# zenghjian/SceneSplat

Measured on AMD Instinct MI355X. Metric: Gaussians/s encoder fwd+bwd, 102k-pt chunks, higher is better.
Workload: dtype bf16

## Files before the change

### include/scenesplat_hip.h

```cpp
#ifndef SCENESPLAT_HIP_H
#define SCENESPLAT_HIP_H
#include <stddef.h>
#include <stdint.h>

#ifdef __cplusplus
extern "C" {
#endif

struct ihipStream_t;
typedef struct ihipStream_t* ss_stream_t;

#define SS_MAX_ORDERS 8
enum { SS_ORDER_Z = 0, SS_ORDER_Z_TRANS = 1, SS_ORDER_HILBERT = 2, SS_ORDER_HILBERT_TRANS = 3 };
enum { SS_DTYPE_F32 = 0, SS_DTYPE_BF16 = 1 };
enum { SS_ATTN_SIMT = 0, SS_ATTN_MFMA = 1 };
enum { SS_OK = 0, SS_ERR_ARG = 1, SS_ERR_LAUNCH = 2, SS_ERR_WORKSPACE = 3 };

int ss_version(void);

int ss_serialize_encode(const int32_t* grid_coord, const int32_t* batch, int64_t n, int depth, const int* orders,
                        int num_orders, int64_t* codes, ss_stream_t stream);
int ss_offsets_to_batch(const int32_t* offsets, int num_batches, int64_t n, int32_t* batch, ss_stream_t stream);
int ss_count_duplicates(const int64_t* sorted_keys, int64_t n, int32_t* count, ss_stream_t stream);
int ss_grid_coord_max(const int32_t* grid_coord, int64_t n, int32_t* out_max, ss_stream_t stream);
// ... 60 lines not shown
size_t ss_window_attn_hm_bwd_workspace_bytes(int64_t n, int64_t n_pad, int channels, int num_heads);
int ss_window_attn_hm_bwd(const void* hm, const void* out, const void* dout, const float* neg_lse2, const int32_t* gidx,
                          const int32_t* sidx, const int32_t* win_start, int num_windows, int max_window, int64_t n,
                          int64_t n_pad, int channels, int num_heads, float scale, void* dqkv, void* workspace,
                          size_t workspace_bytes, ss_stream_t stream);

int ss_window_attn_rpe_fwd(const void* qkv, const int32_t* gidx, const int32_t* sidx, const int32_t* win_start,
                           int num_windows, int max_window, int64_t n, int64_t n_pad, int channels, int num_heads,
                           float scale, int dtype, int impl, const int32_t* grid_coord, const float* table, int pos_bnd,
                           void* out, float* lse, ss_stream_t stream);
size_t ss_window_attn_rpe_bwd_workspace_bytes(int64_t n, int64_t n_pad, int channels, int num_heads, int dtype,
                                              int num_windows, int max_window, int pos_bnd);
int ss_window_attn_rpe_bwd(const void* qkv, const void* out, const void* dout, const float* lse, const int32_t* gidx,
                           const int32_t* sidx, const int32_t* win_start, int num_windows, int max_window, int64_t n,
                           int64_t n_pad, int channels, int num_heads, float scale, int dtype, int impl,
                           const int32_t* grid_coord, const float* table, int pos_bnd, void* dqkv, float* dtable,
                           void* workspace, size_t workspace_bytes, ss_stream_t stream);

int ss_subm_rulebook(const int32_t* grid_coord, const int32_t* batch, int64_t n, int depth,
                     const int64_t* zkeys_sorted, const int32_t* zorder, int swap_xy, int kernel_size, int32_t* nbr,
                     ss_stream_t stream);
int ss_subm_tap_mask_keys(const int32_t* nbr, const int32_t* order, int64_t n, int taps, int coarse_bits, int64_t* keys,
                          ss_stream_t stream);
int64_t ss_subm_rulebook_table_size(int64_t n);
int ss_subm_rulebook_hashed(const int32_t* grid_coord, const int32_t* batch, int64_t n, int depth, int kernel_size, int32_t* nbr,
                            void* workspace, size_t workspace_bytes, ss_stream_t stream);

int ss_subm_conv_fwd(const void* in, const void* weight, const float* bias, const int32_t* nbr, const int32_t* rowperm,
                     void* out, int64_t n, int cin, int cout, int taps, int out_dtype, ss_stream_t stream);
int ss_subm_weight_mirror(const void* w, void* wt, int cout, int taps, int cin, ss_stream_t stream);
int ss_stream_create_cu_mask(int nwords, const uint32_t* mask, void** stream_out);
int ss_subm_im2col(const void* src, const int32_t* nbr, void* dst, int64_t n, int taps, int64_t row_bytes, ss_stream_t stream);
int ss_gemm8_ok(int64_t m, int k, int n, int taps);
int ss_subm_conv_fwd_pipe(const void* in, const void* weight, const float* bias, const int32_t* nbr, const int32_t* rowperm,
                          void* out, int64_t n, int cin, int cout, int taps, int out_dtype, ss_stream_t stream);
int ss_subm_conv_fwd_pipe_walk(const void* in, const void* weight, const float* bias, const int32_t* nbr_walk, const int32_t* rowperm,
                               void* out, int64_t n, int cin, int cout, int taps, int out_dtype, ss_stream_t stream);
int ss_subm_conv_fwd_uses_pipe(int64_t n, int cin, int cout, int taps);
int ss_subm_conv_fwd_walk(const void* in, const void* weight, const float* bias, const int32_t* nbr, const int32_t* nbr_walk,
                          const int32_t* rowperm, void* out, int64_t n, int cin, int cout, int taps, int out_dtype, ss_stream_t stream);
int ss_linear_fwd(const void* x, const void* weight, const float* bias, void* out, int64_t m, int k, int n, int out_dtype,
                  ss_stream_t stream);
int ss_wgrad_xcd_order(void);
int ss_wgrad_set_xcd_order(int on);
int ss_wgrad8_ok(int64_t n, int cin, int cout, int taps);
int ss_subm_conv_wgrad_pipe(const void* in, const void* dout, const int32_t* nbr, const int32_t* rowperm,
                            const int32_t* blk_count, const int32_t* blk_list, float* dweight, int64_t n, int cin, int cout,
                            int taps, ss_stream_t stream);
int ss_linear_wgrad(const void* x, const void* dy, float* dweight, float* dbias, int64_t m, int k_in, int n_out,
                    ss_stream_t stream);
int ss_linear_wgrad_group_plan(int64_t m, int k_in, int n_out, int64_t* desc_words);
int ss_linear_wgrad_tiles(int k_in, int n_out);
int ss_linear_wgrad_group_plan2(int64_t m, int k_in, int n_out, int launch_tiles, int64_t* desc_words);
int ss_linear_wgrad_group(const int64_t* desc, const int32_t* wg_start, int nprob, int total_workgroups, ss_stream_t stream);
int ss_subm_conv_splits(int64_t n, int cout, int taps);
int ss_subm_conv_fwd_splitk(const void* in, const void* weight, const float* bias, const int32_t* nbr, const int32_t* rowperm,
                            float* acc32, int64_t n, int cin, int cout, int taps, int splits, ss_stream_t stream);
int ss_subm_block_lists(const int32_t* nbr, const int32_t* rowperm, int64_t n, int taps, int32_t* blk_count,
                        int32_t* blk_list, ss_stream_t stream);
int ss_subm_conv_wgrad(const void* in, const void* dout, const int32_t* nbr, const int32_t* rowperm,
                       const int32_t* blk_count, const int32_t* blk_list, float* dweight, int64_t n, int cin, int cout,
                       int taps, ss_stream_t stream);

int ss_subm_f32_ok(int cin_padded, int cout);
int ss_subm_f32_fwd(const float* in, const float* wq, const float* bias, const int32_t* nbr_walk, const int32_t* rowperm,
                    float* out, int64_t n, int cin_padded, int cout, int taps, ss_stream_t stream);
int ss_subm_f32_dgrad_dup(const float* dout_folded, const float* wq, const int32_t* nbr_walk, const int32_t* rowperm, float* din,
                          int64_t n, int cin_padded, int cout, int taps, ss_stream_t stream);
int ss_subm_f32_wgrad(const float* in, const float* dout, const int32_t* nbr_walk, const int32_t* rowperm,
                      const int32_t* blk_count, const int32_t* blk_list, float* dweight, int64_t n, int cin_padded,
                      int cin, int cout, int taps, ss_stream_t stream);

int ss_subm_conv_wgrad_pipe_walk(const void* in, const void* dout, const int32_t* nbr_walk, const int32_t* rowperm,
                                 const int32_t* blk_count, const int32_t* blk_list, float* dweight, int64_t n, int cin, int cout,
                                 int taps, ss_stream_t stream);
int ss_subm_conv_wgrad_uses_pipe(int64_t n, int cin, int cout, int taps);
// ... 211 lines not shown
```

### scenesplat_amd/csrc/gemm8.hip

```cpp
#include "common.h"
#include <stdlib.h>

typedef __attribute__((ext_vector_type(8))) __bf16 g8_bf8_t;
#define G8_MFMA(a, b, c) __builtin_amdgcn_mfma_f32_16x16x32_bf16((a), (b), (c), 0, 0, 0)
#define G8_TAPS_MAX 27
#define G8_ZERO_ELEMS 4096

#ifndef G8_STAGGER
#define G8_STAGGER 1
#endif
#define G8_BUF 65536
#define G8_HALF 16384
#define G8_OFF_B 32768
#define G8_OFF_NBR 131072
#define G8_OFF_ROWID (G8_OFF_NBR + G8_TAPS_MAX * 256 * 4)
#define G8_OFF_MASK (G8_OFF_ROWID + 1024)
#define G8_LDS_BYTES (G8_OFF_MASK + 16)

__device__ uint4 g8_zero[G8_ZERO_ELEMS / 8];

__device__ __forceinline__ void g8_glds16(const void* gsrc, char* lds_wave_base) {
  __builtin_amdgcn_global_load_lds((const __attribute__((address_space(1))) void*)gsrc,
                                   (__attribute__((address_space(3))) void*)lds_wave_base, 16, 0, 0);
}
__device__ __forceinline__ g8_bf8_t g8_lds(const char* p) {
  return __builtin_bit_cast(g8_bf8_t, *reinterpret_cast<const uint4*>(p));
}

template <bool GATHER, typename OutT, bool HM = false>
__global__ void __launch_bounds__(512)
k_gemm8(const unsigned short* __restrict__ A, const unsigned short* __restrict__ W, const float* __restrict__ bias,
        const int32_t* __restrict__ nbr, const int32_t* __restrict__ rowperm, OutT* __restrict__ out, int M, int K,
        int N, int taps, int ntn, int hm_c = 0, int hm_d = 0, float hm_scale = 1.f, int walk = 0) {
  __shared__ __attribute__((aligned(16))) char smem[G8_LDS_BYTES];
  int32_t* nbr_s = reinterpret_cast<int32_t*>(smem + G8_OFF_NBR);
  int32_t* rowid_s = reinterpret_cast<int32_t*>(smem + G8_OFF_ROWID);
  unsigned* mask_s = reinterpret_cast<unsigned*>(smem + G8_OFF_MASK);
  const int tid = threadIdx.x, wave = tid >> 6, lane = tid & 63, lq = lane & 15, g = lane >> 4;
  const int wr = wave >> 2, wc = wave & 3;
  int L;
  {
    const int nwg = gridDim.x, orig = blockIdx.x, xcd = orig & 7, q = nwg >> 3, r = nwg & 7;
    L = (xcd < r ? xcd * (q + 1) : r * (q + 1) + (xcd - r) * q) + (orig >> 3);
  }
  const int m0 = (L / ntn) * 256, n0 = (L % ntn) * 256;

  unsigned rem = 0u;
  int tap = 0;
  if (GATHER) {
    if (tid < 256) {
      int k = m0 + tid;
      rowid_s[tid] = k < M ? (rowperm ? rowperm[k] : k) : -1;
    }
    if (tid == 0) *mask_s = 0u;
    __syncthreads();
    constexpr int NIT = (G8_TAPS_MAX * 256 + 511) / 512;
    int vals[NIT];
    const int last = taps * 256 - 1;
#pragma unroll
    for (int it = 0; it < NIT; ++it) {
      const int e = min(it * 512 + tid, last), tt = e >> 8, r = e & 255;
      if (walk) {
        const int k = m0 + r;
        const int v = nbr[(int64_t)tt * M + min(k, M - 1)];
        vals[it] = k < M ? v : -1;
      } else {
        const int row = rowid_s[r];
        const int v = nbr[(int64_t)tt * M + max(row, 0)];
        vals[it] = row >= 0 ? v : -1;
      }
    }
#pragma unroll
    for (int it = 0; it < NIT; ++it) {
      const int e = it * 512 + tid;
      if (e <= last) {
        nbr_s[e] = vals[it];
        if (__ballot(vals[it] >= 0) != 0ULL && lane == 0) atomicOr(mask_s, 1u << (e >> 8));
      }
    }
    __syncthreads();
    rem = __builtin_amdgcn_readfirstlane(*mask_s);
  }
  const int ksteps = K >> 6;
  int T;
  if (GATHER) {
    T = __builtin_popcount(rem) * ksteps;
    if (rem) { tap = __builtin_ctz(rem); rem &= rem - 1u; }
  } else {
    T = ksteps;
  }

  f32x4_t acc[2][4][2][2];
#pragma unroll
  for (int a = 0; a < 2; ++a)
#pragma unroll
    for (int mi = 0; mi < 4; ++mi)
#pragma unroll
      for (int b = 0; b < 2; ++b)
#pragma unroll
        for (int ni = 0; ni < 2; ++ni) acc[a][mi][b][ni] = f32x4_t{0.f, 0.f, 0.f, 0.f};

  const int lc8 = (((tid & 7) ^ ((tid >> 4) & 7)) << 3);
  const int srow = tid >> 3;
  const unsigned short* pA[4];
  const unsigned short* pB[2][2];
  auto load_rows = [&](int tp) {
#pragma unroll
    for (int q = 0; q < 4; ++q) {
      int R = 128 * (q >> 1) + 64 * (q & 1) + srow;
      if (GATHER) {
        int src = nbr_s[tp * 256 + R];
        pA[q] = (src >= 0 ? A + (int64_t)src * K : reinterpret_cast<const unsigned short*>(g8_zero)) + lc8;
      } else {
        int row = min(m0 + R, M - 1);
        if (HM) row = rowperm[row];
        pA[q] = A + (int64_t)row * K + lc8;
      }
    }
  };
#pragma unroll
  for (int h = 0; h < 2; ++h)
#pragma unroll
    for (int j = 0; j < 2; ++j) {
      int col = min(n0 + 128 * j + 64 * (tid >> 8) + 32 * h + (srow & 31), N - 1);
      pB[h][j] = W + (int64_t)col * taps * K + lc8;
    }
  int kc = 0;
  int64_t boff = (int64_t)tap * K;
  load_rows(tap);
  int staged = 0;
  auto advance = [&]() {
    if (staged + 1 >= T) return;
    ++staged;
    kc += 64;
    if (GATHER) {
      if (kc == K) {
        kc = 0;
        tap = __builtin_ctz(rem); rem &= rem - 1u;
        boff = (int64_t)tap * K;
        load_rows(tap);
      }
    } else if (kc == K) {
      kc = 0;
    }
  };
  char* const dst0 = smem + wave * 1024;
  auto stageA = [&](int buf, int h) {
    char* d = dst0 + buf * G8_BUF + h * G8_HALF;
    g8_glds16(pA[h] + kc, d);
    g8_glds16(pA[2 + h] + kc, d + 8192);
  };
  auto stageB = [&](int buf, int h) {
    char* d = dst0 + buf * G8_BUF + G8_OFF_B + h * G8_HALF;
    g8_glds16(pB[h][0] + boff + kc, d);
    g8_glds16(pB[h][1] + boff + kc, d + 8192);
  };

  const int sw = (lq >> 1) & 7;
  const int oA = (wr * 64 + lq) * 128 + ((g ^ sw) << 4);
  const int oB = G8_OFF_B + (wc * 32 + lq) * 128 + ((g ^ sw) << 4);
  g8_bf8_t af[4][2], b0f[2][2], b1f[2][2];
  auto readA = [&](int buf, int h) {
    const char* base = smem + buf * G8_BUF + h * G8_HALF;
#pragma unroll
    for (int mi = 0; mi < 4; ++mi) {
      af[mi][0] = g8_lds(base + oA + mi * 2048);
      af[mi][1] = g8_lds(base + (oA ^ 64) + mi * 2048);
    }
  };
  auto readB = [&](int buf, int h, g8_bf8_t (&bf)[2][2]) {
    const char* base = smem + buf * G8_BUF + h * G8_HALF;
#pragma unroll
    for (int ni = 0; ni < 2; ++ni) {
      bf[ni][0] = g8_lds(base + oB + ni * 2048);
      bf[ni][1] = g8_lds(base + (oB ^ 64) + ni * 2048);
    }
  };
#define G8_MM(HA, HB, BF)                                                                         \
  _Pragma("unroll") for (int ks = 0; ks < 2; ++ks)                                                \
  _Pragma("unroll") for (int mi = 0; mi < 4; ++mi)                                                \
  _Pragma("unroll") for (int ni = 0; ni < 2; ++ni)                                                \
      acc[HA][mi][HB][ni] = G8_MFMA(BF[ni][ks], af[mi][ks], acc[HA][mi][HB][ni]);
#define G8_BAR() do { __builtin_amdgcn_sched_barrier(0); __builtin_amdgcn_s_barrier(); __builtin_amdgcn_sched_barrier(0); } while (0)
#define G8_COMPUTE_BEGIN() do { G8_BAR(); asm volatile("s_waitcnt lgkmcnt(0)" ::: "memory"); __builtin_amdgcn_sched_barrier(0); __builtin_amdgcn_s_setprio(1); } while (0)
#define G8_COMPUTE_END() do { __builtin_amdgcn_s_setprio(0); G8_BAR(); } while (0)

  if (T > 0) {
    stageB(0, 0); stageA(0, 0); stageB(0, 1); stageA(0, 1);
    advance();
    stageB(1, 0); stageA(1, 0); stageB(1, 1);
    asm volatile("s_waitcnt vmcnt(6)" ::: "memory");
    G8_BAR();
#if G8_STAGGER
    if (wr == 1) G8_BAR();
#endif
    for (int t = 0; t < T; ++t) {
      const int buf = t & 1;
      readB(buf, 0, b0f);
      __builtin_amdgcn_sched_barrier(0);
      readA(buf, 0);
      stageA(buf ^ 1, 1);
#if G8_STAGGER
      __builtin_amdgcn_sched_barrier(0);
      asm volatile("s_waitcnt lgkmcnt(8)" ::: "memory");
#endif
      G8_COMPUTE_BEGIN();
      G8_MM(0, 0, b0f)
      G8_COMPUTE_END();
      advance();
      readB(buf, 1, b1f);
      stageB(buf, 0);
      G8_COMPUTE_BEGIN();
      G8_MM(0, 1, b1f)
      G8_COMPUTE_END();
      readA(buf, 1);
      stageA(buf, 0);
      G8_COMPUTE_BEGIN();
      G8_MM(1, 1, b1f)
      G8_COMPUTE_END();
      stageB(buf, 1);
      asm volatile("s_waitcnt vmcnt(6)" ::: "memory");
      G8_COMPUTE_BEGIN();
      G8_MM(1, 0, b0f)
      G8_COMPUTE_END();
    }
#if G8_STAGGER
    if (wr == 0) G8_BAR();
#endif
    asm volatile("s_waitcnt vmcnt(0)" ::: "memory");
  }

  int64_t hm_base[2][2];
  float hm_mul[2][2];
  if (HM) {
#pragma unroll
    for (int hb = 0; hb < 2; ++hb)
#pragma unroll
      for (int ni = 0; ni < 2; ++ni) {
        const int col = min(n0 + 64 * wc + 32 * hb + 16 * ni + 4 * g, N - 4);
        const int sec = col / hm_c, cc = col - sec * hm_c, hd = cc / hm_d, dd = cc - hd * hm_d;
        hm_base[hb][ni] = ((int64_t)sec * (hm_c / hm_d) + hd) * M * hm_d + dd;
        hm_mul[hb][ni] = sec == 0 ? hm_scale : 1.f;
      }
  }
#pragma unroll
  for (int ha = 0; ha < 2; ++ha)
#pragma unroll
    for (int mi = 0; mi < 4; ++mi) {
      const int R = 128 * wr + 64 * ha + 16 * mi + lq;
      int64_t row;
      if (GATHER) { row = rowid_s[R]; } else { row = m0 + R < M ? m0 + R : -1; }
      if (row < 0) continue;
#pragma unroll
      for (int hb = 0; hb < 2; ++hb)
#pragma unroll
        for (int ni = 0; ni < 2; ++ni) {
          const int col = n0 + 64 * wc + 32 * hb + 16 * ni + 4 * g;
          if (col >= N) continue;
          f32x4_t v = acc[ha][mi][hb][ni];
          if (bias) { float4 bv = *reinterpret_cast<const float4*>(bias + col); v[0] += bv.x; v[1] += bv.y; v[2] += bv.z; v[3] += bv.w; }
          OutT* op = out + row * N + col;
          if (HM) {
            const float m_ = hm_mul[hb][ni];
            v[0] *= m_; v[1] *= m_; v[2] *= m_; v[3] *= m_;
            op = out + hm_base[hb][ni] + row * hm_d;
          }
          if (sizeof(OutT) == 2) {
            uint2 u; u.x = pack_bf16x2(v[0], v[1]); u.y = pack_bf16x2(v[2], v[3]);
            *reinterpret_cast<uint2*>(op) = u;
          } else {
            *reinterpret_cast<float4*>(op) = make_float4(v[0], v[1], v[2], v[3]);
          }
        }
    }
}

extern "C" int ss_gemm8_ok(int64_t m, int k, int n, int taps) {
  return m > 0 && m < (1LL << 31) && k >= 64 && (k & 63) == 0 && k <= G8_ZERO_ELEMS && n >= 4 && (n & 3) == 0 &&
         taps >= 1 && taps <= G8_TAPS_MAX;
}

template <bool GATHER>
static int g8_launch(const void* a, const void* w, const float* bias, const int32_t* nbr, const int32_t* rowperm, void* out,
                     int64_t m, int k, int n, int taps, int out_dtype, hipStream_t stream, int walk = 0) {
  if (!ss_gemm8_ok(m, k, n, taps)) return SS_ERR_ARG;
  const int ntm = ss_div_up(m, 256), ntn = ss_div_up(n, 256);
  dim3 grid(ntm * ntn), block(512);
  const unsigned short* A = (const unsigned short*)a; const unsigned short* Wp = (const unsigned short*)w;
  if (out_dtype == SS_BF16)
    SS_LAUNCH((k_gemm8<GATHER, unsigned short>), grid, block, 0, stream, A, Wp, bias, nbr, rowperm, (unsigned short*)out, (int)m, k, n, taps, ntn, 0, 0, 1.f, walk);
  else if (out_dtype == SS_F32)
    SS_LAUNCH((k_gemm8<GATHER, float>), grid, block, 0, stream, A, Wp, bias, nbr, rowperm, (float*)out, (int)m, k, n, taps, ntn, 0, 0, 1.f, walk);
  else
    return SS_ERR_ARG;
  return SS_OK;
}

extern "C" int ss_subm_conv_fwd_pipe(const void* in, const void* weight, const float* bias, const int32_t* nbr,
                                     const int32_t* rowperm, void* out, int64_t n, int cin, int cout, int taps,
                                     int out_dtype, hipStream_t stream) {
  if (n == 0) return SS_OK;
  return g8_launch<true>(in, weight, bias, nbr, rowperm, out, n, cin, cout, taps, out_dtype, stream);
}

extern "C" int ss_subm_conv_fwd_pipe_walk(const void* in, const void* weight, const float* bias, const int32_t* nbr_walk,
                                          const int32_t* rowperm, void* out, int64_t n, int cin, int cout, int taps,
                                          int out_dtype, hipStream_t stream) {
  if (n == 0) return SS_OK;
  return g8_launch<true>(in, weight, bias, nbr_walk, rowperm, out, n, cin, cout, taps, out_dtype, stream, 1);
}

extern "C" int ss_linear_fwd(const void* x, const void* weight, const float* bias, void* out, int64_t m, int k, int n,
                             int out_dtype, hipStream_t stream) {
  if (m == 0) return SS_OK;
  return g8_launch<false>(x, weight, bias, nullptr, nullptr, out, m, k, n, 1, out_dtype, stream);
}

extern "C" int ss_linear_fwd_headmajor(const void* x, const int32_t* row_index, const void* weight, const float* bias,
                                       void* out_hm, int64_t m, int k, int n_out, int channels, int head_dim,
                                       float sec0_scale, hipStream_t stream) {
  if (m == 0) return SS_OK;
  if (!ss_gemm8_ok(m, k, n_out, 1) || channels <= 0 || head_dim <= 0 || (head_dim & 3) || channels % head_dim || n_out % channels ||
      !row_index)
    return SS_ERR_ARG;
  const int ntm = ss_div_up(m, 256), ntn = ss_div_up(n_out, 256);
  dim3 grid(ntm * ntn), block(512);
  SS_LAUNCH((k_gemm8<false, unsigned short, true>), grid, block, 0, stream, (const unsigned short*)x, (const unsigned short*)weight,
            bias, (const int32_t*)nullptr, row_index, (unsigned short*)out_hm, (int)m, k, n_out, 1, ntn, channels, head_dim,
            sec0_scale);
  return SS_OK;
}
```

### scenesplat_amd/native.py

```python
import ctypes

import numpy as np
import torch

from . import _lib, grouped
from ._lib import check

_C = _lib.CONSTANTS
F32, BF16 = _C["SS_DTYPE_F32"], _C["SS_DTYPE_BF16"]
ATTN_SIMT, ATTN_MFMA = _C["SS_ATTN_SIMT"], _C["SS_ATTN_MFMA"]
HAVE_MFMA_ATTN = True
ORDER_IDS = {name: _C["SS_ORDER_" + name.upper().replace("-", "_")] for name in ("z", "z-trans", "hilbert", "hilbert-trans")}


def _p(t):
    return ctypes.c_void_p(t.data_ptr()) if t is not None else ctypes.c_void_p(0)


def _stream():
    return ctypes.c_void_p(torch.cuda.current_stream().cuda_stream)


def _req(t, dtype=None, name="tensor", shape=None):
    if not isinstance(t, torch.Tensor) or not t.is_cuda:
# ... 168 lines not shown
        check(lib().ss_subm_conv_fwd_splitk(_p(x), _p(w), _p(bias), _p(nbr), _p(rowperm), _p(acc), n, cin, cout, taps, splits,
                                            _stream()), "ss_subm_conv_fwd_splitk")
        return acc if out_dtype == torch.float32 else acc.to(out_dtype)
    out = torch.empty((n, cout), dtype=out_dtype, device=x.device)
    if nbr_walk is not None:
        _req(nbr_walk, torch.int32, "nbr_walk", (taps, n))
        check(lib().ss_subm_conv_fwd_walk(_p(x), _p(w), _p(bias), _p(nbr), _p(nbr_walk), _p(rowperm), _p(out), n, cin, cout, taps,
                                          dtype_code(out), _stream()), "ss_subm_conv_fwd_walk")
        return out
    check(lib().ss_subm_conv_fwd(_p(x), _p(w), _p(bias), _p(nbr), _p(rowperm), _p(out), n, cin, cout, taps,
                                 dtype_code(out), _stream()), "ss_subm_conv_fwd")
    return out


def subm_weight_mirror(w):
    cout, taps, cin = w.shape
    _req(w, torch.bfloat16, "w")
    wt = torch.empty((cin, taps, cout), dtype=torch.bfloat16, device=w.device)
    check(lib().ss_subm_weight_mirror(_p(w), _p(wt), cout, taps, cin, _stream()), "ss_subm_weight_mirror")
    return wt


def subm_im2col(x, nbr):
    n, c = x.shape
    taps = nbr.shape[0]
    _req(x, torch.bfloat16, "x"); _req(nbr, torch.int32, "nbr", (taps, n))
    if c % 8:
        raise RuntimeError("subm_im2col: channels must be a multiple of 8")
    out = torch.empty((n, taps * c), dtype=torch.bfloat16, device=x.device)
    check(lib().ss_subm_im2col(_p(x), _p(nbr), _p(out), n, taps, c * 2, _stream()), "ss_subm_im2col")
    return out


def subm_conv_fwd_pipe(x, w, bias, nbr, rowperm, out_dtype=torch.bfloat16):
    n, cin = x.shape
    cout, taps = w.shape[0], w.shape[1]
    out = torch.empty((n, cout), dtype=out_dtype, device=x.device)
    check(lib().ss_subm_conv_fwd_pipe(_p(x), _p(w), _p(bias), _p(nbr), _p(rowperm), _p(out), n, cin, cout, taps,
                                      dtype_code(out), _stream()), "ss_subm_conv_fwd_pipe")
    return out


def linear_fwd(x, w, bias=None, out_dtype=torch.bfloat16):
    m, k = x.shape
    n = w.shape[0]
    out = torch.empty((m, n), dtype=out_dtype, device=x.device)
    check(lib().ss_linear_fwd(_p(x), _p(w), _p(bias), _p(out), m, k, n, dtype_code(out), _stream()), "ss_linear_fwd")
    return out


def subm_block_lists(nbr, rowperm):
    taps, n = nbr.shape
    _req(nbr, torch.int32, "nbr")
    if rowperm is not None:
        _req(rowperm, torch.int32, "rowperm", (n,))
    nb = (n + 63) // 64
    cnt = torch.empty(taps, dtype=torch.int32, device=nbr.device)
    lst = torch.empty((taps, nb), dtype=torch.int32, device=nbr.device)
    check(lib().ss_subm_block_lists(_p(nbr), _p(rowperm), n, taps, _p(cnt), _p(lst), _stream()), "ss_subm_block_lists")
    return cnt, lst


_ARENA = {"buf": None, "off": 0}


def zero_arena_begin(numel, device):
    _ARENA["buf"] = torch.zeros(int(numel), dtype=torch.float32, device=device) if numel > 0 else None
    _ARENA["off"] = 0


def zeros_f32(numel, device):
    buf, off = _ARENA["buf"], _ARENA["off"]
    if buf is not None and buf.device == device and off + numel <= buf.numel():
        _ARENA["off"] = off + ((numel + 3) & ~3)
        return buf[off:off + numel]
    return torch.zeros(int(numel), dtype=torch.float32, device=device)


def subm_conv_wgrad(x, dout, nbr, rowperm, blocks, out=None, nbr_walk=None):
    n, cin = x.shape
    cout = dout.shape[1]
# ... 1354 lines not shown
```

Measured before the change: 2.909 million.

## Add two-phase software-pipelined main loop to gemm8 kernel as default

Adds a PH template parameter to the 256x256 MFMA GEMM kernel and a new two-phase K-loop schedule. Each iteration splits into two compute halves with interleaved LDS reads and global->LDS staging, using fewer barriers than the existing four-phase schedule. The two-phase path becomes the default and the four-phase path stays selectable through an env var or a setter. The different wait counts and stage ordering risk changing latency hiding or exposing more memory stalls.

Result: no change. 2.931 million, median of 6 (+0.7%).

```diff
diff --git a/include/scenesplat_hip.h b/include/scenesplat_hip.h
--- a/include/scenesplat_hip.h
+++ b/include/scenesplat_hip.h
@@ -126,6 +126,7 @@
 int ss_linear_fwd(const void* x, const void* weight, const float* bias, void* out, int64_t m, int k, int n, int out_dtype,
                   ss_stream_t stream);
 int ss_wgrad_xcd_order(void);
+int ss_gemm8_set_phases(int phases);
 int ss_wgrad_set_xcd_order(int on);
 int ss_wgrad8_ok(int64_t n, int cin, int cout, int taps);
 int ss_subm_conv_wgrad_pipe(const void* in, const void* dout, const int32_t* nbr, const int32_t* rowperm,
diff --git a/scenesplat_amd/csrc/gemm8.hip b/scenesplat_amd/csrc/gemm8.hip
--- a/scenesplat_amd/csrc/gemm8.hip
+++ b/scenesplat_amd/csrc/gemm8.hip
@@ -8,6 +8,9 @@
 
 #ifndef G8_STAGGER
 #define G8_STAGGER 1
+#endif
+#ifndef G8_PHASES_DEFAULT
+#define G8_PHASES_DEFAULT 2
 #endif
 #define G8_BUF 65536
 #define G8_HALF 16384
@@ -27,7 +30,7 @@
   return __builtin_bit_cast(g8_bf8_t, *reinterpret_cast<const uint4*>(p));
 }
 
-template <bool GATHER, typename OutT, bool HM = false>
+template <bool GATHER, typename OutT, bool HM = false, int PH = 2>
 __global__ void __launch_bounds__(512)
 k_gemm8(const unsigned short* __restrict__ A, const unsigned short* __restrict__ W, const float* __restrict__ bias,
         const int32_t* __restrict__ nbr, const int32_t* __restrict__ rowperm, OutT* __restrict__ out, int M, int K,
@@ -185,7 +188,7 @@
 #define G8_COMPUTE_BEGIN() do { G8_BAR(); asm volatile("s_waitcnt lgkmcnt(0)" ::: "memory"); __builtin_amdgcn_sched_barrier(0); __builtin_amdgcn_s_setprio(1); } while (0)
 #define G8_COMPUTE_END() do { __builtin_amdgcn_s_setprio(0); G8_BAR(); } while (0)
 
-  if (T > 0) {
+  if (T > 0 && PH == 4) {
     stageB(0, 0); stageA(0, 0); stageB(0, 1); stageA(0, 1);
     advance();
     stageB(1, 0); stageA(1, 0); stageB(1, 1);
@@ -229,6 +232,49 @@
 #endif
     asm volatile("s_waitcnt vmcnt(0)" ::: "memory");
   }
+  if (T > 0 && PH == 2) {
+    stageB(0, 0); stageA(0, 0); stageB(0, 1); stageA(0, 1);
+    advance();
+    stageA(1, 0); stageB(1, 0); stageB(1, 1);
+    asm volatile("s_waitcnt vmcnt(6)" ::: "memory");
+    G8_BAR();
+#if G8_STAGGER
+    if (wr == 1) G8_BAR();
+    if (wr == 1) __builtin_amdgcn_s_setprio(1);
+#endif
+    for (int t = 0; t < T; ++t) {
+      const int buf = t & 1;
+      readB(buf, 0, b0f);
+      readA(buf, 0);
+      readB(buf, 1, b1f);
+      __builtin_amdgcn_sched_barrier(0);
+      stageA(buf ^ 1, 1);
+      __builtin_amdgcn_sched_barrier(0);
+      asm volatile("s_waitcnt vmcnt(8) lgkmcnt(0)" ::: "memory");
+      G8_BAR();
+      G8_MM(0, 0, b0f)
+      G8_MM(0, 1, b1f)
+      G8_BAR();
+      advance();
+      readA(buf, 1);
+      __builtin_amdgcn_sched_barrier(0);
+      stageA(buf, 0);
+      __builtin_amdgcn_sched_barrier(0);
+      stageB(buf, 0);
+      stageB(buf, 1);
+      __builtin_amdgcn_sched_barrier(0);
+      asm volatile("s_waitcnt vmcnt(8) lgkmcnt(0)" ::: "memory");
+      G8_BAR();
+      G8_MM(1, 1, b1f)
+      G8_MM(1, 0, b0f)
+      G8_BAR();
+    }
+#if G8_STAGGER
+    if (wr == 0) G8_BAR();
+    __builtin_amdgcn_s_setprio(0);
+#endif
+    asm volatile("s_waitcnt vmcnt(0)" ::: "memory");
+  }
 
   int64_t hm_base[2][2];
   float hm_mul[2][2];
@@ -280,6 +326,22 @@
          taps >= 1 && taps <= G8_TAPS_MAX;
 }
 
+static int g8_phases_flag = -1;
+static int g8_phases() {
+  if (g8_phases_flag < 0) { const char* e = getenv("SS_GEMM8_PHASES"); g8_phases_flag = (e && atoi(e) == 4) ? 4 : G8_PHASES_DEFAULT; }
+  return g8_phases_flag;
+}
+extern "C" int ss_gemm8_set_phases(int phases) {
+  if (phases != 0 && phases != 2 && phases != 4) return SS_ERR_ARG;
+  g8_phases_flag = phases ? phases : -1;
+  return SS_OK;
+}
+#define G8_LAUNCH_PH(GATHER_, OutT_, HM_, ...)                                                              \
+  do {                                                                                                      \
+    if (g8_phases() == 4) SS_LAUNCH((k_gemm8<GATHER_, OutT_, HM_, 4>), grid, block, 0, stream, __VA_ARGS__); \
+    else SS_LAUNCH((k_gemm8<GATHER_, OutT_, HM_, 2>), grid, block, 0, stream, __VA_ARGS__);                 \
+  } while (0)
+
 template <bool GATHER>
 static int g8_launch(const void* a, const void* w, const float* bias, const int32_t* nbr, const int32_t* rowperm, void* out,
                      int64_t m, int k, int n, int taps, int out_dtype, hipStream_t stream, int walk = 0) {
@@ -288,9 +350,9 @@
   dim3 grid(ntm * ntn), block(512);
   const unsigned short* A = (const unsigned short*)a; const unsigned short* Wp = (const unsigned short*)w;
   if (out_dtype == SS_BF16)
-    SS_LAUNCH((k_gemm8<GATHER, unsigned short>), grid, block, 0, stream, A, Wp, bias, nbr, rowperm, (unsigned short*)out, (int)m, k, n, taps, ntn, 0, 0, 1.f, walk);
+    G8_LAUNCH_PH(GATHER, unsigned short, false, A, Wp, bias, nbr, rowperm, (unsigned short*)out, (int)m, k, n, taps, ntn, 0, 0, 1.f, walk);
   else if (out_dtype == SS_F32)
-    SS_LAUNCH((k_gemm8<GATHER, float>), grid, block, 0, stream, A, Wp, bias, nbr, rowperm, (float*)out, (int)m, k, n, taps, ntn, 0, 0, 1.f, walk);
+    G8_LAUNCH_PH(GATHER, float, false, A, Wp, bias, nbr, rowperm, (float*)out, (int)m, k, n, taps, ntn, 0, 0, 1.f, walk);
   else
     return SS_ERR_ARG;
   return SS_OK;
@@ -325,8 +387,8 @@
     return SS_ERR_ARG;
   const int ntm = ss_div_up(m, 256), ntn = ss_div_up(n_out, 256);
   dim3 grid(ntm * ntn), block(512);
-  SS_LAUNCH((k_gemm8<false, unsigned short, true>), grid, block, 0, stream, (const unsigned short*)x, (const unsigned short*)weight,
-            bias, (const int32_t*)nullptr, row_index, (unsigned short*)out_hm, (int)m, k, n_out, 1, ntn, channels, head_dim,
-            sec0_scale);
+  G8_LAUNCH_PH(false, unsigned short, true, (const unsigned short*)x, (const unsigned short*)weight,
+               bias, (const int32_t*)nullptr, row_index, (unsigned short*)out_hm, (int)m, k, n_out, 1, ntn, channels, head_dim,
+               sec0_scale, 0);
   return SS_OK;
 }
diff --git a/scenesplat_amd/native.py b/scenesplat_amd/native.py
--- a/scenesplat_amd/native.py
+++ b/scenesplat_amd/native.py
@@ -239,6 +239,10 @@
     out = torch.empty((m, n), dtype=out_dtype, device=x.device)
     check(lib().ss_linear_fwd(_p(x), _p(w), _p(bias), _p(out), m, k, n, dtype_code(out), _stream()), "ss_linear_fwd")
     return out
+
+
+def gemm8_set_phases(phases):
+    check(lib().ss_gemm8_set_phases(int(phases)), "ss_gemm8_set_phases")
 
 
 def subm_block_lists(nbr, rowperm):
```

## Add persistent linear GEMM kernel with cross-tile prefetch and split conv path

Applied to the files above, without the earlier changes.

Splits the gemm8 kernel into a gather-conv variant and a dense linear variant. The linear and head-major kernels now run persistently: the grid is capped at the CU count and each workgroup loops over tiles in XCD-aware order. The next tile's loads are staged during the current tile's tail, and row indices and bias are prefetched into LDS via async loads. This is meant to remove launch and tail bubbles and pipeline drains between tiles. The cost is more complex control flow, inline asm LDS reads, and less parallelism when tiles are few.

New measurement: 2.880 million before, 2.894 million after (median of 6 runs). About the same (+0.5%).

```diff
diff --git a/include/scenesplat_hip.h b/include/scenesplat_hip.h
--- a/include/scenesplat_hip.h
+++ b/include/scenesplat_hip.h
@@ -116,6 +116,10 @@
 int ss_stream_create_cu_mask(int nwords, const uint32_t* mask, void** stream_out);
 int ss_subm_im2col(const void* src, const int32_t* nbr, void* dst, int64_t n, int taps, int64_t row_bytes, ss_stream_t stream);
 int ss_gemm8_ok(int64_t m, int k, int n, int taps);
+int ss_gemm8_persistent(void);
+int ss_gemm8_set_persistent(int on);
+int ss_gemm8_max_wgs(void);
+int ss_gemm8_set_max_wgs(int cap);
 int ss_subm_conv_fwd_pipe(const void* in, const void* weight, const float* bias, const int32_t* nbr, const int32_t* rowperm,
                           void* out, int64_t n, int cin, int cout, int taps, int out_dtype, ss_stream_t stream);
 int ss_subm_conv_fwd_pipe_walk(const void* in, const void* weight, const float* bias, const int32_t* nbr_walk, const int32_t* rowperm,
diff --git a/scenesplat_amd/csrc/gemm8.hip b/scenesplat_amd/csrc/gemm8.hip
--- a/scenesplat_amd/csrc/gemm8.hip
+++ b/scenesplat_amd/csrc/gemm8.hip
@@ -16,6 +16,9 @@
 #define G8_OFF_ROWID (G8_OFF_NBR + G8_TAPS_MAX * 256 * 4)
 #define G8_OFF_MASK (G8_OFF_ROWID + 1024)
 #define G8_LDS_BYTES (G8_OFF_MASK + 16)
+#define G8L_OFF_ROWS 131072
+#define G8L_OFF_BIAS (G8L_OFF_ROWS + 2048)
+#define G8L_LDS_BYTES (G8L_OFF_BIAS + 1024)
 
 __device__ uint4 g8_zero[G8_ZERO_ELEMS / 8];
 
@@ -23,15 +26,45 @@
   __builtin_amdgcn_global_load_lds((const __attribute__((address_space(1))) void*)gsrc,
                                    (__attribute__((address_space(3))) void*)lds_wave_base, 16, 0, 0);
 }
+__device__ __forceinline__ void g8_glds4(const void* gsrc, char* lds_wave_base) {
+  __builtin_amdgcn_global_load_lds((const __attribute__((address_space(1))) void*)gsrc,
+                                   (__attribute__((address_space(3))) void*)lds_wave_base, 4, 0, 0);
+}
 __device__ __forceinline__ g8_bf8_t g8_lds(const char* p) {
   return __builtin_bit_cast(g8_bf8_t, *reinterpret_cast<const uint4*>(p));
 }
-
-template <bool GATHER, typename OutT, bool HM = false>
+__device__ __forceinline__ unsigned g8_lds_addr(const void* p) {
+  return (unsigned)(uintptr_t)(const __attribute__((address_space(3))) char*)p;
+}
+__device__ __forceinline__ void g8_lds_read4(const int32_t* base, const int (&idx)[4], int (&v)[4]) {
+  asm volatile("ds_read_b32 %0, %4\n\tds_read_b32 %1, %5\n\tds_read_b32 %2, %6\n\tds_read_b32 %3, %7\n\ts_waitcnt lgkmcnt(0)"
+               : "=&v"(v[0]), "=&v"(v[1]), "=&v"(v[2]), "=&v"(v[3])
+               : "v"(g8_lds_addr(base + idx[0])), "v"(g8_lds_addr(base + idx[1])), "v"(g8_lds_addr(base + idx[2])),
+                 "v"(g8_lds_addr(base + idx[3]))
+               : "memory");
+}
+__device__ __forceinline__ void g8_lds_read4x4(const char* p, f32x4_t (&v)[4]) {
+  asm volatile("ds_read_b128 %0, %4\n\tds_read_b128 %1, %4 offset:64\n\tds_read_b128 %2, %4 offset:128\n\t"
+               "ds_read_b128 %3, %4 offset:192\n\ts_waitcnt lgkmcnt(0)"
+               : "=&v"(v[0]), "=&v"(v[1]), "=&v"(v[2]), "=&v"(v[3])
+               : "v"(g8_lds_addr(p))
+               : "memory");
+}
+template <typename OutT>
+__device__ __forceinline__ void g8_store(OutT* op, f32x4_t v) {
+  if (sizeof(OutT) == 2) {
+    uint2 u; u.x = pack_bf16x2(v[0], v[1]); u.y = pack_bf16x2(v[2], v[3]);
+    *reinterpret_cast<uint2*>(op) = u;
+  } else {
+    *reinterpret_cast<float4*>(op) = make_float4(v[0], v[1], v[2], v[3]);
+  }
+}
+
+template <typename OutT>
 __global__ void __launch_bounds__(512)
-k_gemm8(const unsigned short* __restrict__ A, const unsigned short* __restrict__ W, const float* __restrict__ bias,
-        const int32_t* __restrict__ nbr, const int32_t* __restrict__ rowperm, OutT* __restrict__ out, int M, int K,
-        int N, int taps, int ntn, int hm_c = 0, int hm_d = 0, float hm_scale = 1.f, int walk = 0) {
+k_gemm8_conv(const unsigned short* __restrict__ A, const unsigned short* __restrict__ W, const float* __restrict__ bias,
+             const int32_t* __restrict__ nbr, const int32_t* __restrict__ rowperm, OutT* __restrict__ out, int M, int K,
+             int N, int taps, int ntn, int walk) {
   __shared__ __attribute__((aligned(16))) char smem[G8_LDS_BYTES];
   int32_t* nbr_s = reinterpret_cast<int32_t*>(smem + G8_OFF_NBR);
   int32_t* rowid_s = reinterpret_cast<int32_t*>(smem + G8_OFF_ROWID);
@@ -47,7 +80,7 @@
 
   unsigned rem = 0u;
   int tap = 0;
-  if (GATHER) {
+  {
     if (tid < 256) {
       int k = m0 + tid;
       rowid_s[tid] = k < M ? (rowperm ? rowperm[k] : k) : -1;
@@ -82,13 +115,8 @@
     rem = __builtin_amdgcn_readfirstlane(*mask_s);
   }
   const int ksteps = K >> 6;
-  int T;
-  if (GATHER) {
-    T = __builtin_popcount(rem) * ksteps;
-    if (rem) { tap = __builtin_ctz(rem); rem &= rem - 1u; }
-  } else {
-    T = ksteps;
-  }
+  const int T = __builtin_popcount(rem) * ksteps;
+  if (rem) { tap = __builtin_ctz(rem); rem &= rem - 1u; }
 
   f32x4_t acc[2][4][2][2];
 #pragma unroll
@@ -108,14 +136,8 @@
 #pragma unroll
     for (int q = 0; q < 4; ++q) {
       int R = 128 * (q >> 1) + 64 * (q & 1) + srow;
-      if (GATHER) {
-        int src = nbr_s[tp * 256 + R];
-        pA[q] = (src >= 0 ? A + (int64_t)src * K : reinterpret_cast<const unsigned short*>(g8_zero)) + lc8;
-      } else {
-        int row = min(m0 + R, M - 1);
-        if (HM) row = rowperm[row];
-        pA[q] = A + (int64_t)row * K + lc8;
-      }
+      int src = nbr_s[tp * 256 + R];
+      pA[q] = (src >= 0 ? A + (int64_t)src * K : reinterpret_cast<const unsigned short*>(g8_zero)) + lc8;
     }
   };
 #pragma unroll
@@ -133,15 +155,13 @@
     if (staged + 1 >= T) return;
     ++staged;
     kc += 64;
-    if (GATHER) {
+    {
       if (kc == K) {
         kc = 0;
         tap = __builtin_ctz(rem); rem &= rem - 1u;
         boff = (int64_t)tap * K;
         load_rows(tap);
       }
-    } else if (kc == K) {
-      kc = 0;
     }
   };
   char* const dst0 = smem + wave * 1024;
@@ -230,26 +250,21 @@
     asm volatile("s_waitcnt vmcnt(0)" ::: "memory");
   }
 
-  int64_t hm_base[2][2];
-  float hm_mul[2][2];
-  if (HM) {
-#pragma unroll
-    for (int hb = 0; hb < 2; ++hb)
-#pragma unroll
-      for (int ni = 0; ni < 2; ++ni) {
-        const int col = min(n0 + 64 * wc + 32 * hb + 16 * ni + 4 * g, N - 4);
-        const int sec = col / hm_c, cc = col - sec * hm_c, hd = cc / hm_d, dd = cc - hd * hm_d;
-        hm_base[hb][ni] = ((int64_t)sec * (hm_c / hm_d) + hd) * M * hm_d + dd;
-        hm_mul[hb][ni] = sec == 0 ? hm_scale : 1.f;
-      }
-  }
+  float4 bq[2][2];
+#pragma unroll
+  for (int hb = 0; hb < 2; ++hb)
+#pragma unroll
+    for (int ni = 0; ni < 2; ++ni) {
+      const int col = min(n0 + 64 * wc + 32 * hb + 16 * ni + 4 * g, N - 4);
+      bq[hb][ni] = bias ? *reinterpret_cast<const float4*>(bias + col) : make_float4(0.f, 0.f, 0.f, 0.f);
+    }
 #pragma unroll
   for (int ha = 0; ha < 2; ++ha)
 #pragma unroll
     for (int mi = 0; mi < 4; ++mi) {
       const int R = 128 * wr + 64 * ha + 16 * mi + lq;
       int64_t row;
-      if (GATHER) { row = rowid_s[R]; } else { row = m0 + R < M ? m0 + R : -1; }
+      row = rowid_s[R];
       if (row < 0) continue;
 #pragma unroll
       for (int hb = 0; hb < 2; ++hb)
@@ -258,39 +273,295 @@
           const int col = n0 + 64 * wc + 32 * hb + 16 * ni + 4 * g;
           if (col >= N) continue;
           f32x4_t v = acc[ha][mi][hb][ni];
-          if (bias) { float4 bv = *reinterpret_cast<const float4*>(bias + col); v[0] += bv.x; v[1] += bv.y; v[2] += bv.z; v[3] += bv.w; }
+          if (bias) { const float4 bv = bq[hb][ni]; v[0] += bv.x; v[1] += bv.y; v[2] += bv.z; v[3] += bv.w; }
           OutT* op = out + row * N + col;
-          if (HM) {
-            const float m_ = hm_mul[hb][ni];
-            v[0] *= m_; v[1] *= m_; v[2] *= m_; v[3] *= m_;
-            op = out + hm_base[hb][ni] + row * hm_d;
+          g8_store(op, v);
+        }
+    }
+}
+
+
+template <typename OutT, bool HM>
+__global__ void __launch_bounds__(512)
+k_gemm8_lin(const unsigned short* __restrict__ A, const unsigned short* __restrict__ W, const float* __restrict__ bias,
+            const int32_t* __restrict__ rowperm, OutT* __restrict__ out, int M, int K, int N, int ntn, int ntiles,
+            int hm_c = 0, int hm_d = 0, float hm_scale = 1.f) {
+  __shared__ __attribute__((aligned(16))) char smem[G8L_LDS_BYTES];
+  int32_t* rows_s = reinterpret_cast<int32_t*>(smem + G8L_OFF_ROWS);
+  const int tid = threadIdx.x, wave = tid >> 6, lane = tid & 63, lq = lane & 15, g = lane >> 4;
+  const int wr = wave >> 2, wc = wave & 3;
+  const int nwg = gridDim.x, wg = blockIdx.x;
+  const int ntw = (ntiles - wg + nwg - 1) / nwg;
+  const int xq = ntiles >> 3, xr = ntiles & 7;
+  auto tile_of = [&](int i) {
+    const int v = wg + i * nwg, xcd = v & 7;
+    return (xcd < xr ? xcd * (xq + 1) : xr * (xq + 1) + (xcd - xr) * xq) + (v >> 3);
+  };
+  const int ksteps = K >> 6;
+#define G8_TID(t_) int t_ = threadIdx.x; asm volatile("" : "+v"(t_))
+  f32x4_t acc[2][4][2][2];
+
+  const unsigned short* pA[4] = {A, A, A, A};
+  const unsigned short* pB[2][2] = {{W, W}, {W, W}};
+  const int T = ksteps, Ts = ksteps;
+  int si = 0, m0s = 0, n0s = 0;
+  int staged = 0;
+  int kc = 0;
+  int stopped = 0;
+  auto load_rows = [&]() {
+    G8_TID(t_);
+    const int lc8 = (((t_ & 7) ^ ((t_ >> 4) & 7)) << 3), srow = t_ >> 3;
+#pragma unroll
+    for (int q = 0; q < 4; ++q) {
+      int row = min(m0s + 128 * (q >> 1) + 64 * (q & 1) + srow, M - 1);
+      if (HM) row = rowperm[row];
+      pA[q] = A + (int64_t)row * K + lc8;
+    }
+  };
+  auto load_cols = [&]() {
+    G8_TID(t_);
+    const int lc8 = (((t_ & 7) ^ ((t_ >> 4) & 7)) << 3), srow = t_ >> 3;
+#pragma unroll
+    for (int h = 0; h < 2; ++h)
+#pragma unroll
+      for (int j = 0; j < 2; ++j) {
+        int col = min(n0s + 128 * j + 64 * (t_ >> 8) + 32 * h + (srow & 31), N - 1);
+        pB[h][j] = W + (int64_t)col * K + lc8;
+      }
+  };
+  auto prefetch_rows = [&](int i) {
+    const int m0n = (tile_of(i) / ntn) * 256;
+    G8_TID(t_);
+    if (t_ < 256) g8_glds4(rowperm + min(m0n + t_, M - 1), smem + G8L_OFF_ROWS + (i & 1) * 1024 + (t_ >> 6) * 256);
+  };
+  auto advance = [&]() {
+    if (stopped) return;
+    if (staged + 1 < Ts) {
+      ++staged;
+      kc += 64;
+      return;
+    }
+    if (Ts < 3 || si + 1 >= ntw) { stopped = 1; return; }
+    ++si;
+    const int L = tile_of(si);
+    m0s = (L / ntn) * 256; n0s = (L % ntn) * 256;
+    staged = 0; kc = 0;
+    load_cols();
+    if (HM) {
+      G8_TID(t_);
+      const int sr = t_ >> 3, idx[4] = {sr, 64 + sr, 128 + sr, 192 + sr};
+      int rows[4];
+      g8_lds_read4(rows_s + (si & 1) * 256, idx, rows);
+#pragma unroll
+      for (int q = 0; q < 4; ++q) pA[q] = A + (int64_t)rows[q] * K + (((t_ & 7) ^ ((t_ >> 4) & 7)) << 3);
+      if (si + 1 < ntw) prefetch_rows(si + 1);
+    } else {
+      load_rows();
+    }
+  };
+  char* const dst0 = smem + wave * 1024;
+  auto stageA = [&](int buf, int h) {
+    char* d = dst0 + buf * G8_BUF + h * G8_HALF;
+    g8_glds16(pA[h] + kc, d);
+    g8_glds16(pA[2 + h] + kc, d + 8192);
+  };
+  auto stageB = [&](int buf, int h) {
+    char* d = dst0 + buf * G8_BUF + G8_OFF_B + h * G8_HALF;
+    g8_glds16(pB[h][0] + kc, d);
+    g8_glds16(pB[h][1] + kc, d + 8192);
+  };
+
+  const int sw = (lq >> 1) & 7;
+  const int oA = (wr * 64 + lq) * 128 + ((g ^ sw) << 4);
+  const int oB = G8_OFF_B + (wc * 32 + lq) * 128 + ((g ^ sw) << 4);
+  g8_bf8_t af[4][2], b0f[2][2], b1f[2][2];
+  auto readA = [&](int buf, int h) {
+    const char* base = smem + buf * G8_BUF + h * G8_HALF;
+#pragma unroll
+    for (int mi = 0; mi < 4; ++mi) {
+      af[mi][0] = g8_lds(base + oA + mi * 2048);
+      af[mi][1] = g8_lds(base + (oA ^ 64) + mi * 2048);
+    }
+  };
+  auto readB = [&](int buf, int h, g8_bf8_t (&bf)[2][2]) {
+    const char* base = smem + buf * G8_BUF + h * G8_HALF;
+#pragma unroll
+    for (int ni = 0; ni < 2; ++ni) {
+      bf[ni][0] = g8_lds(base + oB + ni * 2048);
+      bf[ni][1] = g8_lds(base + (oB ^ 64) + ni * 2048);
+    }
+  };
+#define G8_OPAQUE(v) asm volatile("" : "+v"(v))
+
+  int gk = 0;
+  bool fresh = true;
+  for (int ci = 0; ci < ntw; ++ci) {
+    const int Lc = tile_of(ci), m0 = (Lc / ntn) * 256, n0 = (Lc % ntn) * 256;
+    auto stage_bias = [&]() {
+      G8_TID(t_);
+      if (bias && t_ < 256) g8_glds4(bias + min(n0 + t_, N - 1), smem + G8L_OFF_BIAS + (t_ >> 6) * 256);
+    };
+    if (fresh) {
+      __syncthreads();
+      si = ci; m0s = m0; n0s = n0;
+      staged = 0; kc = 0; gk = 0; stopped = 0;
+      stage_bias();
+      load_cols();
+      load_rows();
+      if (HM && ci + 1 < ntw) prefetch_rows(ci + 1);
+      stageB(0, 0); stageA(0, 0); stageB(0, 1); stageA(0, 1);
+      advance();
+      stageB(1, 0); stageA(1, 0); stageB(1, 1);
+      asm volatile("s_waitcnt vmcnt(6)" ::: "memory");
+      G8_BAR();
+#if G8_STAGGER
+      if (wr == 1) G8_BAR();
+#endif
+    }
+#pragma unroll
+    for (int a = 0; a < 2; ++a)
+#pragma unroll
+      for (int mi = 0; mi < 4; ++mi)
+#pragma unroll
+        for (int b = 0; b < 2; ++b)
+#pragma unroll
+          for (int ni = 0; ni < 2; ++ni) acc[a][mi][b][ni] = f32x4_t{0.f, 0.f, 0.f, 0.f};
+    int t = 0;
+    do {
+      const int buf = gk & 1;
+      readB(buf, 0, b0f);
+      __builtin_amdgcn_sched_barrier(0);
+      readA(buf, 0);
+      stageA(buf ^ 1, 1);
+#if G8_STAGGER
+      __builtin_amdgcn_sched_barrier(0);
+      asm volatile("s_waitcnt lgkmcnt(8)" ::: "memory");
+#endif
+      G8_COMPUTE_BEGIN();
+      G8_MM(0, 0, b0f)
+      G8_COMPUTE_END();
+      advance();
+      readB(buf, 1, b1f);
+      stageB(buf, 0);
+      G8_COMPUTE_BEGIN();
+      G8_MM(0, 1, b1f)
+      G8_COMPUTE_END();
+      if (t == 0 && !fresh) stage_bias();
+      __builtin_amdgcn_sched_barrier(0);
+      readA(buf, 1);
+      stageA(buf, 0);
+      G8_COMPUTE_BEGIN();
+      G8_MM(1, 1, b1f)
+      G8_COMPUTE_END();
+      stageB(buf, 1);
+      asm volatile("s_waitcnt vmcnt(6)" ::: "memory");
+      G8_COMPUTE_BEGIN();
+      G8_MM(1, 0, b0f)
+      G8_COMPUTE_END();
+      ++gk;
+    } while (++t < T);
+    const bool cont = si > ci;
+    if (!cont) {
+#if G8_STAGGER
+      if (wr == 0) G8_BAR();
+#endif
+      asm volatile("s_waitcnt vmcnt(0)" ::: "memory");
+    }
+
+    int lq_e = lq, g_e = g, wr_e = wr, wc_e = wc;
+    G8_OPAQUE(lq_e); G8_OPAQUE(g_e); G8_OPAQUE(wr_e); G8_OPAQUE(wc_e);
+    int64_t hm_base[2][2];
+    float hm_mul[2][2];
+    if (HM) {
+#pragma unroll
+      for (int hb = 0; hb < 2; ++hb)
+#pragma unroll
+        for (int ni = 0; ni < 2; ++ni) {
+          const int col = min(n0 + 64 * wc_e + 32 * hb + 16 * ni + 4 * g_e, N - 4);
+          const int sec = col / hm_c, cc = col - sec * hm_c, hd = cc / hm_d, dd = cc - hd * hm_d;
+          hm_base[hb][ni] = ((int64_t)sec * (hm_c / hm_d) + hd) * M * hm_d + dd;
+          hm_mul[hb][ni] = sec == 0 ? hm_scale : 1.f;
+        }
+    }
+    float4 bq[2][2];
+    {
+      f32x4_t bv[4] = {f32x4_t{0.f, 0.f, 0.f, 0.f}, f32x4_t{0.f, 0.f, 0.f, 0.f}, f32x4_t{0.f, 0.f, 0.f, 0.f}, f32x4_t{0.f, 0.f, 0.f, 0.f}};
+      if (bias) g8_lds_read4x4(smem + G8L_OFF_BIAS + (64 * wc_e + 4 * g_e) * 4, bv);
+#pragma unroll
+      for (int hb = 0; hb < 2; ++hb)
+#pragma unroll
+        for (int ni = 0; ni < 2; ++ni) bq[hb][ni] = make_float4(bv[2 * hb + ni][0], bv[2 * hb + ni][1], bv[2 * hb + ni][2], bv[2 * hb + ni][3]);
+    }
+#pragma unroll
+    for (int ha = 0; ha < 2; ++ha)
+#pragma unroll
+      for (int mi = 0; mi < 4; ++mi) {
+        const int R = 128 * wr_e + 64 * ha + 16 * mi + lq_e;
+        int64_t row;
+        row = m0 + R < M ? m0 + R : -1;
+#pragma unroll
+        for (int hb = 0; hb < 2; ++hb)
+#pragma unroll
+          for (int ni = 0; ni < 2; ++ni) {
+            const int col = n0 + 64 * wc_e + 32 * hb + 16 * ni + 4 * g_e;
+            f32x4_t v = acc[ha][mi][hb][ni];
+            if (row < 0 || col >= N) continue;
+            if (bias) { const float4 bv = bq[hb][ni]; v[0] += bv.x; v[1] += bv.y; v[2] += bv.z; v[3] += bv.w; }
+            OutT* op = out + row * N + col;
+            if (HM) {
+              const float m_ = hm_mul[hb][ni];
+              v[0] *= m_; v[1] *= m_; v[2] *= m_; v[3] *= m_;
+              op = out + hm_base[hb][ni] + row * hm_d;
+            }
+            g8_store(op, v);
           }
-          if (sizeof(OutT) == 2) {
-            uint2 u; u.x = pack_bf16x2(v[0], v[1]); u.y = pack_bf16x2(v[2], v[3]);
-            *reinterpret_cast<uint2*>(op) = u;
-          } else {
-            *reinterpret_cast<float4*>(op) = make_float4(v[0], v[1], v[2], v[3]);
-          }
-        }
-    }
-}
+      }
+    fresh = !cont;
+  }
+}
+
 
 extern "C" int ss_gemm8_ok(int64_t m, int k, int n, int taps) {
   return m > 0 && m < (1LL << 31) && k >= 64 && (k & 63) == 0 && k <= G8_ZERO_ELEMS && n >= 4 && (n & 3) == 0 &&
          taps >= 1 && taps <= G8_TAPS_MAX;
 }
 
-template <bool GATHER>
-static int g8_launch(const void* a, const void* w, const float* bias, const int32_t* nbr, const int32_t* rowperm, void* out,
-                     int64_t m, int k, int n, int taps, int out_dtype, hipStream_t stream, int walk = 0) {
+static int g8_persist_flag = -1, g8_max_wgs = -1;
+extern "C" int ss_gemm8_persistent(void) {
+  if (g8_persist_flag < 0) { const char* e = getenv("SS_GEMM8_PERSISTENT"); g8_persist_flag = (e && atoi(e) == 0) ? 0 : 1; }
+  return g8_persist_flag;
+}
+extern "C" int ss_gemm8_set_persistent(int on) { g8_persist_flag = on ? 1 : 0; return SS_OK; }
+extern "C" int ss_gemm8_max_wgs(void) {
+  if (g8_max_wgs < 0) { const char* e = getenv("SS_GEMM8_MAX_WGS"); g8_max_wgs = (e && atoi(e) > 0) ? atoi(e) : 0; }
+  return g8_max_wgs;
+}
+extern "C" int ss_gemm8_set_max_wgs(int cap) { g8_max_wgs = cap > 0 ? cap : 0; return SS_OK; }
+
+static int g8_grid(int tiles) {
+  if (!ss_gemm8_persistent()) return tiles;
+  int cap = ss_gemm8_max_wgs();
+  if (cap <= 0) {
+    static int cus[64];
+    int dev = 0;
+    if (hipGetDevice(&dev) != hipSuccess || dev < 0 || dev >= 64) return 0;
+    if (cus[dev] <= 0 && (hipDeviceGetAttribute(&cus[dev], hipDeviceAttributeMultiprocessorCount, dev) != hipSuccess || cus[dev] <= 0))
+      return 0;
+    cap = cus[dev];
+  }
+  return tiles < cap ? tiles : cap;
+}
+
+static int g8_launch_conv(const void* a, const void* w, const float* bias, const int32_t* nbr, const int32_t* rowperm, void* out,
+                          int64_t m, int k, int n, int taps, int out_dtype, hipStream_t stream, int walk) {
   if (!ss_gemm8_ok(m, k, n, taps)) return SS_ERR_ARG;
   const int ntm = ss_div_up(m, 256), ntn = ss_div_up(n, 256);
   dim3 grid(ntm * ntn), block(512);
   const unsigned short* A = (const unsigned short*)a; const unsigned short* Wp = (const unsigned short*)w;
   if (out_dtype == SS_BF16)
-    SS_LAUNCH((k_gemm8<GATHER, unsigned short>), grid, block, 0, stream, A, Wp, bias, nbr, rowperm, (unsigned short*)out, (int)m, k, n, taps, ntn, 0, 0, 1.f, walk);
+    SS_LAUNCH((k_gemm8_conv<unsigned short>), grid, block, 0, stream, A, Wp, bias, nbr, rowperm, (unsigned short*)out, (int)m, k, n, taps, ntn, walk);
   else if (out_dtype == SS_F32)
-    SS_LAUNCH((k_gemm8<GATHER, float>), grid, block, 0, stream, A, Wp, bias, nbr, rowperm, (float*)out, (int)m, k, n, taps, ntn, 0, 0, 1.f, walk);
+    SS_LAUNCH((k_gemm8_conv<float>), grid, block, 0, stream, A, Wp, bias, nbr, rowperm, (float*)out, (int)m, k, n, taps, ntn, walk);
   else
     return SS_ERR_ARG;
   return SS_OK;
@@ -300,20 +571,31 @@
                                      const int32_t* rowperm, void* out, int64_t n, int cin, int cout, int taps,
                                      int out_dtype, hipStream_t stream) {
   if (n == 0) return SS_OK;
-  return g8_launch<true>(in, weight, bias, nbr, rowperm, out, n, cin, cout, taps, out_dtype, stream);
+  return g8_launch_conv(in, weight, bias, nbr, rowperm, out, n, cin, cout, taps, out_dtype, stream, 0);
 }
 
 extern "C" int ss_subm_conv_fwd_pipe_walk(const void* in, const void* weight, const float* bias, const int32_t* nbr_walk,
                                           const int32_t* rowperm, void* out, int64_t n, int cin, int cout, int taps,
                                           int out_dtype, hipStream_t stream) {
   if (n == 0) return SS_OK;
-  return g8_launch<true>(in, weight, bias, nbr_walk, rowperm, out, n, cin, cout, taps, out_dtype, stream, 1);
+  return g8_launch_conv(in, weight, bias, nbr_walk, rowperm, out, n, cin, cout, taps, out_dtype, stream, 1);
 }
 
 extern "C" int ss_linear_fwd(const void* x, const void* weight, const float* bias, void* out, int64_t m, int k, int n,
                              int out_dtype, hipStream_t stream) {
   if (m == 0) return SS_OK;
-  return g8_launch<false>(x, weight, bias, nullptr, nullptr, out, m, k, n, 1, out_dtype, stream);
+  if (!ss_gemm8_ok(m, k, n, 1)) return SS_ERR_ARG;
+  const int ntm = ss_div_up(m, 256), ntn = ss_div_up(n, 256), tiles = ntm * ntn, wgs = g8_grid(tiles);
+  if (wgs <= 0) return SS_ERR_LAUNCH;
+  dim3 grid(wgs), block(512);
+  const unsigned short* A = (const unsigned short*)x; const unsigned short* Wp = (const unsigned short*)weight;
+  if (out_dtype == SS_BF16)
+    SS_LAUNCH((k_gemm8_lin<unsigned short, false>), grid, block, 0, stream, A, Wp, bias, (const int32_t*)nullptr, (unsigned short*)out, (int)m, k, n, ntn, tiles, 0, 0, 1.f);
+  else if (out_dtype == SS_F32)
+    SS_LAUNCH((k_gemm8_lin<float, false>), grid, block, 0, stream, A, Wp, bias, (const int32_t*)nullptr, (float*)out, (int)m, k, n, ntn, tiles, 0, 0, 1.f);
+  else
+    return SS_ERR_ARG;
+  return SS_OK;
 }
 
 extern "C" int ss_linear_fwd_headmajor(const void* x, const int32_t* row_index, const void* weight, const float* bias,
@@ -323,10 +605,10 @@
   if (!ss_gemm8_ok(m, k, n_out, 1) || channels <= 0 || head_dim <= 0 || (head_dim & 3) || channels % head_dim || n_out % channels ||
       !row_index)
     return SS_ERR_ARG;
-  const int ntm = ss_div_up(m, 256), ntn = ss_div_up(n_out, 256);
-  dim3 grid(ntm * ntn), block(512);
-  SS_LAUNCH((k_gemm8<false, unsigned short, true>), grid, block, 0, stream, (const unsigned short*)x, (const unsigned short*)weight,
-            bias, (const int32_t*)nullptr, row_index, (unsigned short*)out_hm, (int)m, k, n_out, 1, ntn, channels, head_dim,
-            sec0_scale);
+  const int ntm = ss_div_up(m, 256), ntn = ss_div_up(n_out, 256), tiles = ntm * ntn, wgs = g8_grid(tiles);
+  if (wgs <= 0) return SS_ERR_LAUNCH;
+  dim3 grid(wgs), block(512);
+  SS_LAUNCH((k_gemm8_lin<unsigned short, true>), grid, block, 0, stream, (const unsigned short*)x, (const unsigned short*)weight, bias,
+            row_index, (unsigned short*)out_hm, (int)m, k, n_out, ntn, tiles, channels, head_dim, sec0_scale);
   return SS_OK;
 }
diff --git a/scenesplat_amd/native.py b/scenesplat_amd/native.py
--- a/scenesplat_amd/native.py
+++ b/scenesplat_amd/native.py
@@ -224,13 +224,25 @@
     return out
 
 
-def subm_conv_fwd_pipe(x, w, bias, nbr, rowperm, out_dtype=torch.bfloat16):
+def subm_conv_fwd_pipe(x, w, bias, nbr, rowperm, out_dtype=torch.bfloat16, nbr_walk=None):
     n, cin = x.shape
     cout, taps = w.shape[0], w.shape[1]
     out = torch.empty((n, cout), dtype=out_dtype, device=x.device)
+    if nbr_walk is not None:
+        check(lib().ss_subm_conv_fwd_pipe_walk(_p(x), _p(w), _p(bias), _p(nbr_walk), _p(rowperm), _p(out), n, cin, cout, taps,
+                                               dtype_code(out), _stream()), "ss_subm_conv_fwd_pipe_walk")
+        return out
     check(lib().ss_subm_conv_fwd_pipe(_p(x), _p(w), _p(bias), _p(nbr), _p(rowperm), _p(out), n, cin, cout, taps,
                                       dtype_code(out), _stream()), "ss_subm_conv_fwd_pipe")
     return out
+
+
+def gemm8_set_persistent(on):
+    check(lib().ss_gemm8_set_persistent(1 if on else 0), "ss_gemm8_set_persistent")
+
+
+def gemm8_set_max_wgs(cap):
+    check(lib().ss_gemm8_set_max_wgs(int(cap or 0)), "ss_gemm8_set_max_wgs")
 
 
 def linear_fwd(x, w, bias=None, out_dtype=torch.bfloat16):
```
